# Guoxs/DODT

Measured on AMD Instinct MI355X. Metric: frame-pairs/sec (whole node) KITTI-shape tau=2, higher is better.
Workload: dtype f32

## Files before the change

dodt_amd/_lib.py:

```python
import ctypes as C
import os

_HERE = os.path.dirname(os.path.abspath(__file__))
LIB_PATH = os.environ.get('DODT_HIP_LIB') or os.path.join(_HERE, 'lib', 'libdodt_hip.so')

OK, ERR_INVALID, ERR_HIP, ERR_UNSUPPORTED = 0, 1, 2, 3
PTS_VELO_XYZI, PTS_CAM_3XN = 0, 1
EXTRACTOR_VGG_PYR = 0
EXTRACTOR_VGG = 1
EXTRACTOR_SHARED_GPU = 0x100
EXTRACTOR_BF16 = 0x200
EXTRACTOR_SPLIT = 0x400
FC_RELU = 1
FC_BF16 = 2
CONFLICT_RAISE, CONFLICT_NEXT_BEST = 0, 1


class DodtError(RuntimeError):
    pass


class BevParams(C.Structure):
    _fields_ = [
        ('point_format', C.c_int32),
# ... 82 lines not shown
                                      _pf, _pf, _pf]),
    'dodt_project_anchors_f32': (_i, [_vp, _pf, _i, _pi32, C.POINTER(_f),
                                      C.POINTER(_f), _f, _f, _pf, _pf, _pf]),
    'dodt_img_preprocess': (_i, [_vp, _vp, _i, _i, _i, _i, _i,
                                 C.POINTER(_f), _pf]),
    'dodt_conv_mode': (_i, []),
    'dodt_extractor_create': (_i, [_vp, _i, _i, _i, _i, _i, _i,
                                   C.POINTER(_vp)]),
    'dodt_extractor_destroy': (_i, [_vp]),
    'dodt_extractor_set_layer': (_i, [_vp, C.c_char_p, _vp, _i, _i, _i, _i,
                                      _vp, _vp, _vp]),
    'dodt_extractor_input': (_i, [_vp, C.POINTER(_vp), C.POINTER(C.c_longlong)]),
    'dodt_extractor_forward': (_i, [_vp, _pf, _pf, _pf]),
    'dodt_extractor_forward_padded': (_i, [_vp, _pf, _pf, _pf]),
    'dodt_extractor_set_input': (_i, [_vp, _pf]),
    'dodt_extractor_set_input_support': (_i, [_vp, _vp, _i, _i, C.POINTER(C.c_longlong)]),
    'dodt_extractor_set_frame_tables': (_i, [_vp, _i, C.POINTER(_i)]),
    'dodt_extractor_frame_items': (_i, [_vp, C.POINTER(_i), _i]),
    'dodt_extractor_frame_split': (_i, [_vp, C.POINTER(_i), C.POINTER(_i), _i]),
    'dodt_extractor_store_bytes': (C.c_longlong, [_vp]),
    'dodt_frame_tables_host': (_i, [_vp, _i, _i, _i, _i, _i, _i, _vp, _i, _vp, _vp, C.POINTER(_i)]),
    'dodt_frame_restore_host': (_i, [_vp, _i, _i, _i, _i, _i, _i, _i, _i, _i, _vp, _vp, _vp, _vp]),
    'dodt_frame_lists_host': (_i, [_vp, _i, _i, _i, _i, _i, _i, _vp, _i, _vp, _vp, C.POINTER(_i), _vp, C.POINTER(_i)]),
    'dodt_extractor_read_activation': (_i, [_vp, C.c_char_p, _vp,
                                            C.POINTER(_i), C.POINTER(_i),
                                            C.POINTER(_i)]),
    'dodt_extractor_output_shape': (_i, [_vp, C.POINTER(_i), C.POINTER(_i), C.POINTER(_i)]),
    'dodt_extractor_first_layers_folded': (_i, [_vp]),
    'dodt_extractor_flops': (_d, [_vp]),
    'dodt_extractor_mfma_flops': (_d, [_vp]),
    'dodt_extractor_bytes': (_d, [_vp]),
    'dodt_extractor_layer_count': (_i, [_vp]),
    'dodt_conv_variant_count': (_i, []),
    'dodt_conv_variant_info': (_i, [_i, C.POINTER(ConvVariant)]),
    'dodt_conv_plan_host': (_i, [_i, _i, _i, _i, _i, _i, _i, C.POINTER(ConvLayerPlan), _i, C.POINTER(_i)]),
    'dodt_extractor_layer_plan': (_i, [_vp, C.POINTER(ConvLayerPlan), _i, C.POINTER(_i)]),
    'dodt_extractor_forward_timed': (_i, [_vp, _pf, _pf, _pf, C.POINTER(LayerInfo), _i]),
    'dodt_crop_and_resize': (_i, [_vp, _pf, _i, _i, _i, _pf, _i, _pi32, _i, _i,
                                  _pf]),
    'dodt_crop_and_resize_strided': (_i, [_vp, _pf, _i, _i, _i, _pf, _i, _pi32, _i, _i, _pf,
                                          C.c_longlong]),
    'dodt_correlation': (_i, [_vp, _pf, _pf, _i, _i, _i, _i, _i, _i, _pf]),
    'dodt_crop_and_resize_indexed': (_i, [_vp, _pf, _i, _i, _i, _pf, _i, _pi32, _i, _pi32, _i, _i, _pf,
                                          C.c_longlong]),
    'dodt_correlation_tile_list': (_i, [_vp, _i, _i, _pf, _i, _pi32, _i, _pi32, _i, _i, _pi32, _i, _pi32]),
    'dodt_correlation_tiles': (_i, [_vp, _pf, _pf, _i, _i, _i, _i, _i, _i, _pi32, _i, _pi32, _pf]),
    'dodt_mean_fusion': (_i, [_vp, _pf, _pf, _i, _pi32, _i, _pf]),
    'dodt_fc_create': (_i, [_vp, _i, _i, _hf, _hf, _i, C.POINTER(_vp)]),
    'dodt_fc_create_ex': (_i, [_vp, _i, _i, _hf, _hf, _i, C.POINTER(_vp)]),
    'dodt_fc_destroy': (_i, [_vp]),
    'dodt_fc_forward': (_i, [_vp, _vp, _pf, _pf, _i, _i, _pi32, _pf, _i]),
    'dodt_fc_forward_split': (_i, [_vp, _vp, _pf, _i, _i, _pi32, _i, C.POINTER(_i), C.POINTER(_vp)]),
    'dodt_fc_flops': (_d, [_vp, _i]),
    'dodt_fc_bf16_row_elems': (_i, [_vp]),
    'dodt_fc_forward_bf16': (_i, [_vp, _vp, _vp, _i, _i, _pi32, _vp, _i, _i]),
    'dodt_fc_forward_split_bf16': (_i, [_vp, _vp, _vp, _i, _i, _pi32, _i, C.POINTER(_i), C.POINTER(_vp)]),
    'dodt_rows_to_bf16': (_i, [_vp, _pf, _pf, _i, _pi32, _i, _i, _vp, _i]),
    'dodt_nms': (_i, [_vp, _pf, _pf, _i, _pi32, _i, _f, _pi32, _pi32]),
    'dodt_offset_to_anchor': (_i, [_vp, _pf, _pf, _i, _pi32, _pf]),
    'dodt_softmax_fg': (_i, [_vp, _pf, _i, _pi32, _pf]),
    'dodt_rpn_decode': (_i, [_vp, _pf, _pf, _pf, _i, _pi32, C.POINTER(_f), _pf, _pf, _pf]),
    'dodt_gather_project': (_i, [_vp, _pf, _pi32, _i, _pi32, C.POINTER(_f), C.POINTER(_f), _f, _f, _pf, _pf, _pf]),
    'dodt_final_decode': (_i, [_vp, _pf, _pf, _pf, _pf, _i, _pi32, C.POINTER(_f), C.POINTER(_f),
                               _pf, _pf, _pf, _pf, _pf, _pf]),
    'dodt_gather_rows': (_i, [_vp, _pf, _i, _pi32, _i, _pi32, _pf]),
    'dodt_max_fg_logit': (_i, [_vp, _pf, _i, _i, _pi32, _pf]),
    'dodt_pack_detections': (_i, [_vp, _pf, _pf, _pf, _pf, _pi32, _pi32, _i, _f, _pf, _pi32]),
    'dodt_pack_detections_compact': (_i, [_vp, _pf, _pf, _pf, _pf, _pi32, _pi32, _i, _f, _pf, _pi32]),
    'dodt_angle_vector_to_orientation': (_i, [_vp, _pf, _i, _pi32, _pf]),
    'dodt_class_scores': (_i, [_vp, _pf, _i, _i, _pi32, _pf, _pi32]),
    'dodt_final_decode_classes': (_i, [_vp, _pf, _pf, _pf, _i, _pf, _i, _pi32, C.POINTER(_f), C.POINTER(_f),
                                       _pf, _pf, _pf, _pf, _pf, _pi32, _pf]),
    'dodt_pack_detections_classes': (_i, [_vp, _pf, _pf, _pi32, _pf, _pf, _pi32, _pi32, _i, _f, _pf, _pi32]),
    'dodt_pack_detections_compact_classes': (_i, [_vp, _pf, _pf, _pi32, _pf, _pf, _pi32, _pi32, _i, _f, _pf, _pi32]),
    'dodt_box_4c_decode': (_i, [_vp, _pf, _pf, _i, _pi32, C.POINTER(_f),
                                C.POINTER(_f), _pf, _pf, _pf]),
    'dodt_comm_unique_id': (_i, [_vp]),
    'dodt_comm_create': (_i, [_vp, _i, _i, _vp, C.POINTER(_vp)]),
    'dodt_comm_destroy': (_i, [_vp]),
    'dodt_comm_attach': (_i, [_vp, _vp]),
    'dodt_comm_rank': (_i, [_vp, C.POINTER(_i), C.POINTER(_i)]),
    'dodt_comm_set_late_peer': (_i, [_vp, _d]),
    'dodt_all_gather_records': (_i, [_vp, _vp, _i, _pf, _pi32, _i, _i, _i, _i, _pf, _pi32]),
    'dodt_comm_join': (_i, [_vp, _i, _vp]),
    'dodt_comm_sync': (_i, [_vp]),
    'dodt_comm_barrier': (_i, [_vp]),
    'dodt_comm_max_f64': (_i, [_vp, C.POINTER(_d)]),
    'dodt_three_d_iou_matrix': (_i, [_vp, _vp, _i, _vp, _i, _vp]),
    'dodt_interpolate_pairs': (_i, [_vp, _vp, _i, _pi32, _i, _i, _i, _d, _i, _vp, C.POINTER(_d), _i, _vp,
                                    _pi32, _pi32]),
    'dodt_track_state_bytes': (_i, [_i, C.POINTER(C.c_size_t)]),
    'dodt_track_reset': (_i, [_vp, _vp, _i]),
    'dodt_track_flush': (_i, [_vp, _vp, _d, _i]),
    'dodt_track_encode': (_i, [_vp, _vp, _i, _pi32, _i, _i, C.POINTER(_d), _d, _d, _d, _pf, _pf, _pi32]),
    'dodt_track_pairs': (_i, [_vp, _vp, _vp, _i, _pi32, _i, _i, C.POINTER(_d), _d, _d, _d, _d, _d, _i]),
    'dodt_track_encoded': (_i, [_vp, _vp, _pf, _pf, _pi32, _i, _i, _d, _d, _i]),
}
COMM_ID_BYTES = 128

_lib = None


def load():
    global _lib
    if _lib is not None:
        return _lib
# ... 21 lines not shown
```

dodt_amd/csrc/gemm.hip:

```cpp
#include <cmath>
#include <cstdlib>
#include <mutex>
#include <set>
#include <type_traits>
#include <vector>

#include <algorithm>

#include "common.h"
#include "lds_dma.h"

namespace {

typedef float f32x16 __attribute__((ext_vector_type(16)));
typedef float f32x4 __attribute__((ext_vector_type(4)));

constexpr int kKAlign = 64;
constexpr int kSmallK = 16;

struct GemmArgs {
    const float* x;
    const float* x2;
    const float* w;
    const float* bias;
// ... 347 lines not shown
                wf[q][nt] = *reinterpret_cast<const f32x4*>(sS + w_base + q * (2 * kDmaBN * 4) + nt * 128);
            if (FUSE) x2[q] = *reinterpret_cast<const f32x4*>(sS + kDmaXFloats + xo[q]);
        };
        read_q(0);
        read_q(1);
        __builtin_amdgcn_sched_barrier(0);
        constexpr int kPerQ = (kPerStage + 3) / 4;
#pragma unroll
        for (int q = 0; q < 4; ++q) {
            if (q + 2 < 4) read_q(q + 2);
            if (FUSE) {
#pragma unroll
                for (int e = 0; e < 4; ++e) xf[q][e] = (xf[q][e] + x2[q][e]) / 2.0f;
            }
#pragma unroll
            for (int s2 = 0; s2 < 4; ++s2)
#pragma unroll
                for (int nt = 0; nt < NT; ++nt)
                    acc[nt] = __builtin_amdgcn_mfma_f32_32x32x2f32(xf[q][s2], wf[q][nt][s2], acc[nt], 0, 0, 0);
            if (more) {
#pragma unroll
                for (int n = q * kPerQ; n < (q + 1) * kPerQ && n < kPerStage; ++n) issue_one(st + 2, (BUF + 2) % kDmaStages, n);
            }
            __builtin_amdgcn_sched_barrier(0);
        }
    };
    auto issue = [&](int st, int buf) {
#pragma unroll
        for (int n = 0; n < kPerStage; ++n) issue_one(st, buf, n);
    };
    issue(0, 0);
    if (nstages > 1) issue(1, 1);
    for (int st = 0; st < nstages; st += 3) {
        stage(std::integral_constant<int, 0>{}, st);
        if (st + 1 < nstages) stage(std::integral_constant<int, 1>{}, st + 1);
        if (st + 2 < nstages) stage(std::integral_constant<int, 2>{}, st + 2);
    }
#pragma unroll
    for (int nt = 0; nt < NT; ++nt) {
        const int n = n0 + wn * 32 * NT + nt * 32 + li;
        store_tile32<false>(a, acc[nt], a.bias[n], m0 + wm * 32 + 4 * lh, n, M);
    }
}

int launch_fc_dma(hipStream_t s, const GemmArgs& a, int Npad, int nt) {
    const int tiles_m = dodt::ceil_div(a.M, kDmaBM), tiles_n = Npad / (64 * nt);
    const dim3 grid(tiles_m * tiles_n);
    const size_t x_floats = (size_t)kDmaXFloats * (a.x2 ? 2 : 1);
    const size_t lds = kDmaStages * (x_floats + (size_t)kDmaBK * 64 * nt) * sizeof(float);
    hipError_t e;
    if (a.x2) e = launch_with_lds(&fc_dma_kernel<true, 1>, grid, lds, s, a, tiles_m, tiles_n);
    else if (nt == 2) e = launch_with_lds(&fc_dma_kernel<false, 2>, grid, lds, s, a, tiles_m, tiles_n);
    else e = launch_with_lds(&fc_dma_kernel<false, 1>, grid, lds, s, a, tiles_m, tiles_n);
    DODT_HIP_CHECK(e);
    DODT_LAUNCH_CHECK();
    return DODT_OK;
}

constexpr int kBfBM = 64, kBfBN = 128, kBfStages = 3;
__host__ __device__ constexpr int bf_swz(int r, int S) { return (r / (16 / S)) & (S - 1); }

template <bool YBF16, int BK>
__global__ void __launch_bounds__(256, 2)
fc_bf16_dma_kernel(const GemmArgs a, int tiles_m, int tiles_n) {
    static_assert(kBfStages == 3, "the stage loop is unrolled for a ring of three");
    using dodt::i32x4_t;
    using dodt::kOob;
    using dodt::make_rsrc;
    constexpr int S = BK / 8;
    constexpr int kXBytes = kBfBM * BK * 2, kWBytes = kBfBN * BK * 2, kStage = kXBytes + kWBytes;
    constexpr int kXPieces = kXBytes / 1024 / 4, kWPieces = kWBytes / 1024 / 4;
    constexpr int kPerStage = kXPieces + kWPieces;
    static_assert(kPerStage <= 63, "vmcnt is six bits");
    constexpr int kRowsPerPiece = 1024 / (BK * 2);
    constexpr int NQ = BK / 16;
    extern __shared__ __attribute__((aligned(16))) float smem[];
    const int tid = threadIdx.x, lane = tid & 63;
    const int wave = __builtin_amdgcn_readfirstlane(tid >> 6);
    const int wm = wave >> 1, wn = wave & 1;
    const int li = lane & 31, lh = lane >> 5;
    const int tile = xcd_tile(tiles_m * tiles_n);
    const int mt = tile / tiles_n, nt0 = tile % tiles_n;
    const int m0 = mt * kBfBM;
    const int M = resolved_rows(a.d_m, a.M);
    if (m0 >= M) return;
    const int nstages = a.Kp / BK;
    const int rows = min(M - m0, kBfBM);
    const unsigned short* x16 = reinterpret_cast<const unsigned short*>(a.x);
    const i32x4_t x_rsrc = make_rsrc(x16 + (size_t)m0 * a.ldx, (unsigned)(((size_t)(rows - 1) * a.ldx + a.Kp) * 2));
    const char* wblk = reinterpret_cast<const char*>(a.w) + (size_t)nt0 * nstages * kWBytes;
    const i32x4_t w_rsrc = make_rsrc(wblk, (unsigned)((size_t)nstages * kWBytes));
    int x_off[kXPieces];
#pragma unroll
    for (int k = 0; k < kXPieces; ++k) {
        const int row = (wave + 4 * k) * kRowsPerPiece + lane / S, slot = (lane % S) ^ bf_swz(row, S);
        x_off[k] = row < rows ? (row * a.ldx + slot * 8) * 2 : kOob;
    }
    const int w_off = lane * 16;
    const unsigned lds0 = (unsigned)(size_t)(__attribute__((address_space(3))) void*)smem;
    auto issue_one = [&](int st, int buf, int n) {
        const unsigned sX = lds0 + (unsigned)(buf * kStage);
        if (n < kXPieces) dodt::blds16s(x_rsrc, x_off[n < kXPieces ? n : 0], st * (BK * 2), sX + (unsigned)(wave + 4 * n) * 1024);
        else dodt::blds16s(w_rsrc, w_off, st * kWBytes + (wave + 4 * (n - kXPieces)) * 1024,
                           sX + kXBytes + (unsigned)(wave + 4 * (n - kXPieces)) * 1024);
    };
    f32x16 acc[2];
// ... 284 lines not shown
                t = a[(size_t)r * in_ld + c + e];
                if (b) t = (t + b[(size_t)r * in_ld + c + e]) / 2.0f;
            }
            v[e] = t;
        }
        f32x2 o = {pack_bf16(v[0], v[1]), pack_bf16(v[2], v[3])};
        *reinterpret_cast<f32x2*>(out + (size_t)r * out_ld + c) = o;
    }
}
}

extern "C" int dodt_rows_to_bf16(dodt_ctx* ctx, const float* d_a, const float* d_b, int rows, const int32_t* d_n,
                                 int row_floats, int in_ld, void* d_out_bf16, int out_ld) {
    DODT_REQUIRE(ctx && d_a && d_out_bf16, "dodt_rows_to_bf16: NULL argument");
    DODT_REQUIRE(rows >= 0 && row_floats >= 1 && in_ld >= row_floats && out_ld >= row_floats && out_ld % 4 == 0,
                 "dodt_rows_to_bf16: rows of %d floats, %d apart, into rows of %d bf16 (a multiple of 4)", row_floats,
                 in_ld, out_ld);
    DODT_REQUIRE((size_t)d_out_bf16 % 8 == 0, "dodt_rows_to_bf16: 8-byte aligned output");
    if (rows == 0) return DODT_OK;
    const long long total = (long long)rows * (out_ld / 4);
    const int blocks = (int)std::min<long long>((total + 255) / 256, 4096);
    hipLaunchKernelGGL(rows_to_bf16_kernel, dim3(blocks), dim3(256), 0, ctx->stream, d_a, d_b, rows, d_n, row_floats,
                       in_ld, reinterpret_cast<unsigned short*>(d_out_bf16), out_ld);
    DODT_LAUNCH_CHECK();
    return DODT_OK;
}

struct dodt_fc {
    dodt_ctx* ctx = nullptr;
    int K = 0, Kp = 0, N = 0, Npad = 0, BN = 0, relu = 0;
    bool bf16 = false;
    float* d_w = nullptr;
    float* d_b = nullptr;
    float* d_w_plain = nullptr;
    void* d_w_dma = nullptr;
    int Kd = 0;
    int dma_bk = 0;
    bool smallk = false;
    bool skinny = false;
    bool dma = false;
};

namespace {

enum class FcForm {
    kNone,
    kSmallK,
    kSkinny,
    kSkinnyBf16,
    kSkinnyBf16Rows,
    kDmaNt1,
    kDmaNt2,
    kDmaFused,
    kBf16RowsDma32,
    kBf16RowsDma64,
    kTiled64x128,
    kTiled128x32,
    kTiled64x128Bf16,
    kTiled128x32Bf16,
};

FcForm select_fc_form(const dodt_fc& f, const GemmArgs& a, bool x_bf16, bool y_bf16) {
    if (x_bf16) {
        if (f.d_w_dma) return f.dma_bk == 64 ? FcForm::kBf16RowsDma64 : FcForm::kBf16RowsDma32;
        if (f.skinny && a.ldx % 4 == 0 && (size_t)a.x % 8 == 0 && !y_bf16) return FcForm::kSkinnyBf16Rows;
        return FcForm::kNone;
    }
    if (f.smallk && (size_t)a.y % 16 == 0) return FcForm::kSmallK;
    if (f.skinny && a.ldx % 4 == 0 && (size_t)a.x % 16 == 0 && !a.x2) return f.bf16 ? FcForm::kSkinnyBf16 : FcForm::kSkinny;
    if (f.bf16) {
        return f.BN == 128 ? FcForm::kTiled64x128Bf16 : FcForm::kTiled128x32Bf16;
    }
    if (f.BN != 128) return FcForm::kTiled128x32;
    if (f.dma && a.ldx % 4 == 0 && (size_t)a.x % 16 == 0 && (!a.x2 || (size_t)a.x2 % 16 == 0)) {
        if (a.x2) return FcForm::kDmaFused;
        const long tiles128 = (long)dodt::ceil_div(a.M, kDmaBM) * (f.Npad / 128);
        return tiles128 >= 2 * 256 ? FcForm::kDmaNt2 : FcForm::kDmaNt1;
    }
    return FcForm::kTiled64x128;
}

int launch_fc_form(FcForm form, const dodt_fc& f, hipStream_t s, GemmArgs a, const SplitOut& so, bool y_bf16) {
    switch (form) {
    case FcForm::kSmallK: return launch_fc_smallk(s, a, f.d_w_plain, f.bf16);
    case FcForm::kSkinny: return launch_fc_skinny(s, a, so, false, false);
    case FcForm::kSkinnyBf16: return launch_fc_skinny(s, a, so, true, false);
    case FcForm::kSkinnyBf16Rows: return launch_fc_skinny(s, a, so, true, true);
    case FcForm::kDmaNt1:
    case FcForm::kDmaFused: return launch_fc_dma(s, a, f.Npad, 1);
    case FcForm::kDmaNt2: return launch_fc_dma(s, a, f.Npad, 2);
    case FcForm::kBf16RowsDma32:
    case FcForm::kBf16RowsDma64:
        a.w = reinterpret_cast<const float*>(f.d_w_dma);
        a.Kp = f.Kd;
        return launch_fc_bf16_dma(s, a, f.Npad, y_bf16, f.dma_bk);
    case FcForm::kTiled64x128: return launch_fc<64, 128, 2, 2, 64, false>(s, a, f.Npad);
    case FcForm::kTiled128x32: return launch_fc<128, 32, 4, 1, 32, false>(s, a, f.Npad);
    case FcForm::kTiled64x128Bf16: return launch_fc<64, 128, 2, 2, 32, true>(s, a, f.Npad);
    case FcForm::kTiled128x32Bf16: return launch_fc<128, 32, 4, 1, 64, true>(s, a, f.Npad);
    case FcForm::kNone: break;
    }
    dodt::set_error("dodt_fc: no kernel form selected");
    return DODT_ERR_UNSUPPORTED;
}

GemmArgs fc_args(const dodt_fc& f, const void* d_x, const float* d_x2, int ldx, int M, const int32_t* d_m, void* d_y,
                 int ldy) {
    GemmArgs a;
    a.x = reinterpret_cast<const float*>(d_x); a.x2 = d_x2; a.w = f.d_w; a.bias = f.d_b; a.y = reinterpret_cast<float*>(d_y);
    a.M = M; a.K = f.K; a.Kp = f.Kp; a.N = f.N; a.ldx = ldx; a.ldy = ldy; a.relu = f.relu;
    a.d_m = d_m;
    return a;
}

SplitOut whole_out(const dodt_fc& f, void* d_y, int ldy) {
    float* y = reinterpret_cast<float*>(d_y);
    return SplitOut{{y, y, y}, {f.N, f.N, f.N}, {ldy, ldy, ldy}};
}

int split_out(const char* who, const dodt_fc& f, int parts, const int* widths, float* const* d_ys, SplitOut* so) {
    int end = 0;
    for (int p = 0; p < 3; ++p) {
        const int q = p < parts ? p : parts - 1;
        DODT_REQUIRE(widths[q] >= 1 && d_ys[q], "%s: part %d is empty", who, q);
        if (p < parts) end += widths[p];
        so->y[p] = d_ys[q];
        so->n_end[p] = p < parts ? end : f.N + 1;
        so->ld[p] = widths[q];
    }
    DODT_REQUIRE(end == f.N, "%s: the parts have %d columns, the layer %d", who, end, f.N);
    return DODT_OK;
}

}

extern "C" {

int dodt_fc_create(dodt_ctx* ctx, int K, int N, const float* w, const float* bias, int relu,
                   dodt_fc** out) {
    return dodt_fc_create_ex(ctx, K, N, w, bias, relu ? DODT_FC_RELU : 0, out);
}

int dodt_fc_create_ex(dodt_ctx* ctx, int K, int N, const float* w, const float* bias, int flags,
// ... 107 lines not shown
        dodt::set_error("dodt_fc_forward_split: layers with N <= 32, K %% 16 == 0 and 16-byte aligned rows only");
        return DODT_ERR_UNSUPPORTED;
    }
    if (M == 0) return DODT_OK;
    return launch_fc_form(form, *f, (ctx ? ctx : f->ctx)->stream, a, so, false);
}

int dodt_fc_bf16_row_elems(const dodt_fc* f) {
    if (!f || !f->bf16) return 0;
    if (f->d_w_dma) return f->Kd;
    return f->skinny ? f->K : 0;
}

int dodt_fc_forward_bf16(dodt_fc* f, dodt_ctx* ctx, const void* d_x_bf16, int ldx, int M, const int32_t* d_m,
                         void* d_y, int ldy, int y_bf16) {
    DODT_REQUIRE(f && d_x_bf16 && d_y, "dodt_fc_forward_bf16: NULL argument");
    DODT_REQUIRE(f->bf16, "dodt_fc_forward_bf16: the layer was not created with DODT_FC_BF16");
    DODT_REQUIRE(M >= 0 && ldy >= f->N, "dodt_fc_forward_bf16: bad strides");
    if (M == 0) return DODT_OK;
    const GemmArgs a = fc_args(*f, d_x_bf16, nullptr, ldx, M, d_m, d_y, ldy);
    const FcForm form = select_fc_form(*f, a, true, y_bf16 != 0);
    if (form == FcForm::kBf16RowsDma32 || form == FcForm::kBf16RowsDma64) {
        DODT_REQUIRE(ldx >= f->Kd && ldx % 8 == 0 && (size_t)d_x_bf16 % 16 == 0,
                     "dodt_fc_forward_bf16: rows of >= %d bf16 (zeros beyond K = %d), 16-byte aligned", f->Kd, f->K);
        DODT_REQUIRE((size_t)M * ldx * 2 < (1ull << 31), "dodt_fc_forward_bf16: x block beyond 2 GB");
    } else if (form == FcForm::kSkinnyBf16Rows) {
        DODT_REQUIRE(ldx >= f->K, "dodt_fc_forward_bf16: bad strides");
    } else {
        dodt::set_error("dodt_fc_forward_bf16: layers with N %% 128 == 0 and K >= 128, or N <= 32 and K %% 16 == 0 with "
                        "float32 output, only (K = %d, N = %d)", f->K, f->N);
        return DODT_ERR_UNSUPPORTED;
    }
    return launch_fc_form(form, *f, (ctx ? ctx : f->ctx)->stream, a, whole_out(*f, d_y, ldy), y_bf16 != 0);
}

int dodt_fc_forward_split_bf16(dodt_fc* f, dodt_ctx* ctx, const void* d_x_bf16, int ldx, int M, const int32_t* d_m,
                               int parts, const int* widths, float* const* d_ys) {
    DODT_REQUIRE(f && d_x_bf16 && widths && d_ys, "dodt_fc_forward_split_bf16: NULL argument");
    DODT_REQUIRE(f->bf16, "dodt_fc_forward_split_bf16: the layer was not created with DODT_FC_BF16");
    DODT_REQUIRE(parts >= 1 && parts <= 3, "dodt_fc_forward_split_bf16: %d parts (1..3)", parts);
    DODT_REQUIRE(M >= 0 && ldx >= f->K, "dodt_fc_forward_split_bf16: bad strides");
    const GemmArgs a = fc_args(*f, d_x_bf16, nullptr, ldx, M, d_m, nullptr, 0);
    SplitOut so;
    if (int rc = split_out("dodt_fc_forward_split_bf16", *f, parts, widths, d_ys, &so)) return rc;
    const FcForm form = select_fc_form(*f, a, true, false);
    if (form != FcForm::kSkinnyBf16Rows) {
        dodt::set_error("dodt_fc_forward_split_bf16: layers with N <= 32, K %% 16 == 0 and 8-byte aligned rows only");
        return DODT_ERR_UNSUPPORTED;
    }
    if (M == 0) return DODT_OK;
    return launch_fc_form(form, *f, (ctx ? ctx : f->ctx)->stream, a, so, false);
}

double dodt_fc_flops(const dodt_fc* f, int M) {
    return f ? 2.0 * M * (double)f->K * f->N : 0.0;
}

}
```

dodt_amd/ops.py:

```python
import ctypes as C

import numpy as np

from dodt_amd import _lib


def _arr(ctype, values):
    values = [float(v) for v in np.asarray(values, dtype=np.float64).reshape(-1)]
    return (ctype * len(values))(*values)


def _p(a):
    return None if a is None else C.c_void_p(a.ptr)


def make_bev_params(cfg, velo_to_cam=None, p2=None, im_wh=None,
                    point_format=_lib.PTS_VELO_XYZI, ground_plane=None,
                    area_extents=None, voxel_size=None):
    bp = _lib.BevParams()
    bp.point_format = point_format
    bp.num_slices = int(cfg['num_slices'])
    m = np.zeros(12) if velo_to_cam is None else \
        np.asarray(velo_to_cam, dtype=np.float64).reshape(-1)[:12]
    p = np.zeros(12) if p2 is None else np.asarray(p2, dtype=np.float64).reshape(-1)
# ... 307 lines not shown

    def __init__(self, ctx, w, b, relu, dtype='f32'):
        if dtype not in ('f32', 'bf16'):
            raise ValueError("dtype must be 'f32' or 'bf16'")
        w = np.ascontiguousarray(w, dtype=np.float32)
        b = np.ascontiguousarray(b, dtype=np.float32)
        if w.ndim != 2 or b.shape != (w.shape[1],):
            raise ValueError('weights must be (K,N) and bias (N,)')
        self.ctx, self.K, self.N, self.dtype = ctx, int(w.shape[0]), int(w.shape[1]), dtype
        h = C.c_void_p()
        flags = (_lib.FC_RELU if relu else 0) | (_lib.FC_BF16 if dtype == 'bf16' else 0)
        _lib.check(ctx.lib.dodt_fc_create_ex(ctx.handle, self.K, self.N,
                                             w.ctypes.data_as(C.c_void_p),
                                             b.ctypes.data_as(C.c_void_p), flags, C.byref(h)),
                   'dodt_fc_create_ex')
        self.handle = h

    def forward(self, d_x, M, d_y, ldx=None, ldy=None, d_x2=None, d_m=None, ctx=None):
        c = ctx or self.ctx
        _lib.check(c.lib.dodt_fc_forward(
            self.handle, c.handle, _p(d_x), _p(d_x2), int(self.K if ldx is None else ldx),
            int(M), _p(d_m), _p(d_y), int(self.N if ldy is None else ldy)), 'dodt_fc_forward')

    def can_split(self, ldx=None):
        return self.N <= 32 and self.K % 16 == 0 and (self.K if ldx is None else ldx) % 4 == 0

    def forward_split(self, d_x, M, d_ys, widths, ldx=None, d_m=None, ctx=None):
        c = ctx or self.ctx
        w = (C.c_int * len(widths))(*[int(v) for v in widths])
        ys = (C.c_void_p * len(d_ys))(*[_p(y) for y in d_ys])
        _lib.check(c.lib.dodt_fc_forward_split(
            self.handle, c.handle, _p(d_x), int(self.K if ldx is None else ldx), int(M), _p(d_m),
            len(widths), w, ys), 'dodt_fc_forward_split')

    def bf16_row_elems(self):
        return int(self.ctx.lib.dodt_fc_bf16_row_elems(self.handle)) if self.dtype == 'bf16' else 0

    def forward_bf16(self, d_x, M, d_y, ldx, ldy=None, d_m=None, y_bf16=True, ctx=None):
        c = ctx or self.ctx
        _lib.check(c.lib.dodt_fc_forward_bf16(self.handle, c.handle, _p(d_x), int(ldx), int(M), _p(d_m), _p(d_y),
                                              int(self.N if ldy is None else ldy), 1 if y_bf16 else 0),
                   'dodt_fc_forward_bf16')

    def forward_split_bf16(self, d_x, M, d_ys, widths, ldx, d_m=None, ctx=None):
        c = ctx or self.ctx
        w = (C.c_int * len(widths))(*[int(v) for v in widths])
        ys = (C.c_void_p * len(d_ys))(*[_p(y) for y in d_ys])
        _lib.check(c.lib.dodt_fc_forward_split_bf16(
            self.handle, c.handle, _p(d_x), int(ldx), int(M), _p(d_m), len(widths), w, ys), 'dodt_fc_forward_split_bf16')

    def flops(self, M):
        return 2.0 * M * self.K * self.N

    def close(self):
        if self.handle is not None:
            self.ctx.lib.dodt_fc_destroy(self.handle)
            self.handle = None


def three_d_iou_matrix(ctx, d_a, na, d_b, nb, d_iou_out):
    _lib.check(ctx.lib.dodt_three_d_iou_matrix(ctx.handle, _p(d_a), int(na), _p(d_b), int(nb), _p(d_iou_out)),
               'dodt_three_d_iou_matrix')


def temporal_calib(r0_rect, tr_velo_to_cam):
    r0 = np.asarray(r0_rect, np.float64).reshape(3, 3)
    tr = np.asarray(tr_velo_to_cam, np.float64).reshape(3, 4)
    inv = np.zeros_like(tr)
    inv[0:3, 0:3] = np.transpose(tr[0:3, 0:3])
    inv[0:3, 3] = np.dot(-np.transpose(tr[0:3, 0:3]), tr[0:3, 3])
    return np.concatenate([np.linalg.inv(r0).reshape(-1), inv.reshape(-1), tr.reshape(-1), r0.reshape(-1)])


def temporal_ego(ego, n_frames):
    if len(ego) != n_frames - 1:
        raise ValueError('recovery needs one (trans, matrix, delta) per frame 1..n_frames-1')
    out = np.zeros((n_frames, 13))
    for i, (trans, matrix, delta) in enumerate(ego):
        out[i + 1, 0:3] = np.asarray(trans, np.float64).reshape(3)
        out[i + 1, 3:12] = np.linalg.inv(np.asarray(matrix, np.float64).reshape(3, 3)).reshape(-1)
        out[i + 1, 12] = float(delta)
    return out


def interpolate_pairs(ctx, d_records, d_counts, n_pairs, max_det, n_frames, threshold, on_conflict, d_out,
                      d_out_counts, d_status, d_recover=None, calib=None, max_out=None):
    if on_conflict not in ('raise', 'next_best'):
        raise ValueError("on_conflict must be 'raise' or 'next_best'")
    if d_records.dtype not in (np.float32, np.float64):
        raise ValueError('records must be float32 or float64')
    cal = None if calib is None else _arr(C.c_double, calib)
    _lib.check(ctx.lib.dodt_interpolate_pairs(
        ctx.handle, _p(d_records), int(d_records.dtype == np.float64), _p(d_counts), int(n_pairs), int(max_det),
        int(n_frames), float(threshold), _lib.CONFLICT_NEXT_BEST if on_conflict == 'next_best' else _lib.CONFLICT_RAISE,
        _p(d_recover), cal, int(2 * max_det if max_out is None else max_out), _p(d_out), _p(d_out_counts),
        _p(d_status)), 'dodt_interpolate_pairs')


def track_state_bytes(log_capacity):
    n = C.c_size_t()
    _lib.check(_lib.load().dodt_track_state_bytes(int(log_capacity), C.byref(n)), 'dodt_track_state_bytes')
    return int(n.value)


def track_reset(ctx, d_state, log_capacity):
    _lib.check(ctx.lib.dodt_track_reset(ctx.handle, _p(d_state), int(log_capacity)), 'dodt_track_reset')
# ... 31 lines not shown
```

include/dodt_hip.h:

```cpp
#ifndef DODT_HIP_H
#define DODT_HIP_H

#include <stddef.h>
#include <stdint.h>

#ifdef __cplusplus
extern "C" {
#endif

#define DODT_OK 0
#define DODT_ERR_INVALID 1
#define DODT_ERR_HIP 2
#define DODT_ERR_UNSUPPORTED 3

typedef struct dodt_ctx dodt_ctx;

int dodt_version(void);
const char* dodt_last_error(void);
int dodt_ctx_create(int device_id, dodt_ctx** out);
int dodt_ctx_create_high_priority(int device_id, dodt_ctx** out);
int dodt_ctx_create_on_stream(int device_id, void* hip_stream, dodt_ctx** out);
int dodt_ctx_destroy(dodt_ctx* ctx);
int dodt_ctx_set_plan_cus(dodt_ctx* ctx, int n);
int dodt_ctx_sync(dodt_ctx* ctx);
// ... 147 lines not shown
    int32_t pool_fused;
    int32_t bneck_fused;
    int32_t folded;
    int32_t reserved_;
} dodt_conv_layer_plan;
int dodt_conv_plan_host(int kind, int in_h, int in_w, int in_c, int pad_top, int batch, int num_cus,
                        dodt_conv_layer_plan* out, int n_out, int* n_layers);
int dodt_extractor_layer_plan(const dodt_extractor* ex, dodt_conv_layer_plan* out, int n_out, int* n_layers);
int dodt_extractor_forward_timed(dodt_extractor* ex, const float* d_in, float* d_feat_out,
                                 float* d_bottleneck_out, dodt_layer_info* info, int n_info);

int dodt_crop_and_resize(dodt_ctx* ctx, const float* d_image, int H, int W, int C,
                         const float* d_boxes, int n, const int32_t* d_n, int crop_h,
                         int crop_w, float* d_out);
int dodt_crop_and_resize_strided(dodt_ctx* ctx, const float* d_image, int H, int W, int C,
                                 const float* d_boxes, int n, const int32_t* d_n, int crop_h,
                                 int crop_w, float* d_out, long long out_box_stride);
int dodt_crop_and_resize_indexed(dodt_ctx* ctx, const float* d_image, int H, int W, int C,
                                 const float* d_boxes, int n_boxes, const int32_t* d_box_idx, int n,
                                 const int32_t* d_n, int crop_h, int crop_w, float* d_out,
                                 long long out_box_stride);

int dodt_correlation(dodt_ctx* ctx, const float* d_a, const float* d_b, int H, int W, int C,
                     int max_displacement, int stride_2, int pad, float* d_out);
int dodt_correlation_tile_list(dodt_ctx* ctx, int OH, int OW, const float* d_boxes, int n_boxes,
                               const int32_t* d_box_idx, int n, const int32_t* d_n, int crop_h, int crop_w,
                               int32_t* d_tiles, int capacity, int32_t* d_n_tiles);
int dodt_correlation_tiles(dodt_ctx* ctx, const float* d_a, const float* d_b, int H, int W, int C,
                           int max_displacement, int stride_2, int pad, const int32_t* d_tiles, int capacity,
                           const int32_t* d_n_tiles, float* d_out);

int dodt_mean_fusion(dodt_ctx* ctx, const float* d_a, const float* d_b, int rows, const int32_t* d_n,
                     int row_floats, float* d_out);
typedef struct dodt_fc dodt_fc;
int dodt_fc_create(dodt_ctx* ctx, int K, int N, const float* w, const float* bias, int relu,
                   dodt_fc** out);
#define DODT_FC_RELU 1
#define DODT_FC_BF16 2
int dodt_fc_create_ex(dodt_ctx* ctx, int K, int N, const float* w, const float* bias, int flags,
                      dodt_fc** out);
int dodt_fc_destroy(dodt_fc* fc);
int dodt_fc_forward(dodt_fc* fc, dodt_ctx* ctx, const float* d_x, const float* d_x2, int ldx,
                    int M, const int32_t* d_m, float* d_y, int ldy);
int dodt_fc_forward_split(dodt_fc* fc, dodt_ctx* ctx, const float* d_x, int ldx, int M, const int32_t* d_m,
                          int parts, const int* widths, float* const* d_ys);
int dodt_fc_bf16_row_elems(const dodt_fc* fc);
int dodt_fc_forward_bf16(dodt_fc* fc, dodt_ctx* ctx, const void* d_x_bf16, int ldx, int M, const int32_t* d_m,
                         void* d_y, int ldy, int y_bf16);
int dodt_fc_forward_split_bf16(dodt_fc* fc, dodt_ctx* ctx, const void* d_x_bf16, int ldx, int M, const int32_t* d_m,
                               int parts, const int* widths, float* const* d_ys);
int dodt_rows_to_bf16(dodt_ctx* ctx, const float* d_a, const float* d_b, int rows, const int32_t* d_n,
                      int row_floats, int in_ld, void* d_out_bf16, int out_ld);
double dodt_fc_flops(const dodt_fc* fc, int M);

int dodt_nms(dodt_ctx* ctx, const float* d_boxes, const float* d_scores, int n,
             const int32_t* d_n, int max_out, float iou_threshold, int32_t* d_sel_out,
             int32_t* d_count_out);

int dodt_offset_to_anchor(dodt_ctx* ctx, const float* d_anchors, const float* d_offsets,
                          int n, const int32_t* d_n, float* d_out);
int dodt_softmax_fg(dodt_ctx* ctx, const float* d_logits2, int n, const int32_t* d_n,
                    float* d_scores_out);
int dodt_rpn_decode(dodt_ctx* ctx, const float* d_anchors, const float* d_offsets, const float* d_logits2, int n,
                    const int32_t* d_n, const float bev_extents[4], float* d_regressed_out,
                    float* d_bev_norm_tf_out, float* d_scores_out);
int dodt_gather_project(dodt_ctx* ctx, const float* d_src, const int32_t* d_idx, int n, const int32_t* d_n,
                        const float bev_extents[4], const float p2[12], float im_w, float im_h,
                        float* d_rows_out, float* d_bev_norm_tf_out, float* d_img_norm_tf_out);
int dodt_final_decode(dodt_ctx* ctx, const float* d_top_anchors, const float* d_offsets, const float* d_cls_logits2,
                      const float* d_angle_vectors, int n, const int32_t* d_n, const float plane[4],
                      const float bev_extents[4], float* d_boxes_3d_out, float* d_pred_anchors_out,
                      float* d_bev_tf_out, float* d_nms_scores_out, float* d_det_scores_out,
                      float* d_orientations_out);
int dodt_gather_rows(dodt_ctx* ctx, const float* d_src, int width, const int32_t* d_idx,
                     int n, const int32_t* d_n, float* d_out);
int dodt_max_fg_logit(dodt_ctx* ctx, const float* d_logits, int n_cls, int n,
                      const int32_t* d_n, float* d_scores_out);
int dodt_angle_vector_to_orientation(dodt_ctx* ctx, const float* d_angle_vectors, int n,
                                     const int32_t* d_n, float* d_orientations_out);
int dodt_pack_detections(dodt_ctx* ctx, const float* d_boxes_3d, const float* d_scores,
                         const float* d_orientations, const float* d_corr_offsets,
                         const int32_t* d_sel, const int32_t* d_count, int max_det,
                         float frame_mark, float* d_rec_out, int32_t* d_count_out);
int dodt_pack_detections_compact(dodt_ctx* ctx, const float* d_boxes_3d, const float* d_scores,
                                 const float* d_orientations, const float* d_det_offsets,
                                 const int32_t* d_sel, const int32_t* d_count, int max_det,
                                 float frame_mark, float* d_rec_out, int32_t* d_count_out);
int dodt_class_scores(dodt_ctx* ctx, const float* d_logits, int n_cls, int n, const int32_t* d_n,
                      float* d_scores_out, int32_t* d_types_out);
int dodt_final_decode_classes(dodt_ctx* ctx, const float* d_top_anchors, const float* d_offsets,
                              const float* d_cls_logits, int n_cls, const float* d_angle_vectors, int n,
                              const int32_t* d_n, const float plane[4], const float bev_extents[4],
                              float* d_boxes_3d_out, float* d_pred_anchors_out, float* d_bev_tf_out,
                              float* d_nms_scores_out, float* d_det_scores_out, int32_t* d_det_types_out,
                              float* d_orientations_out);
int dodt_pack_detections_classes(dodt_ctx* ctx, const float* d_boxes_3d, const float* d_scores, const int32_t* d_types,
                                 const float* d_orientations, const float* d_corr_offsets, const int32_t* d_sel,
                                 const int32_t* d_count, int max_det, float frame_mark, float* d_rec_out,
                                 int32_t* d_count_out);
int dodt_pack_detections_compact_classes(dodt_ctx* ctx, const float* d_boxes_3d, const float* d_scores,
                                         const int32_t* d_types, const float* d_orientations,
                                         const float* d_det_offsets, const int32_t* d_sel, const int32_t* d_count,
                                         int max_det, float frame_mark, float* d_rec_out, int32_t* d_count_out);
int dodt_box_4c_decode(dodt_ctx* ctx, const float* d_top_anchors, const float* d_offsets,
                       int n, const int32_t* d_n, const float plane[4],
                       const float bev_extents[4], float* d_boxes_3d_out,
// ... 46 lines not shown
```

Measured before the change: 420.8.

## Add small-M DMA FC kernel tiling N into 16-wide blocks

Adds an f32 FC kernel for M up to 128 rows. It launches one workgroup per 16 output columns, streams X and W through a four-stage LDS ring using buffer-to-LDS DMA, and runs 16x16x4 f32 MFMAs. Form selection now routes unfused DMA-eligible calls with small M to this kernel. The goal is to fill the GPU with many more workgroups than the 64-row tiled DMA path gives for small batches. In exchange, each block re-reads the whole X slab and the waitcnt bookkeeping is hand-tuned. A form-name query is also exposed for diagnostics.

```diff
diff --git a/dodt_amd/_lib.py b/dodt_amd/_lib.py
--- a/dodt_amd/_lib.py
+++ b/dodt_amd/_lib.py
@@ -158,6 +158,7 @@
     'dodt_fc_forward': (_i, [_vp, _vp, _pf, _pf, _i, _i, _pi32, _pf, _i]),
     'dodt_fc_forward_split': (_i, [_vp, _vp, _pf, _i, _i, _pi32, _i, C.POINTER(_i), C.POINTER(_vp)]),
     'dodt_fc_flops': (_d, [_vp, _i]),
+    'dodt_fc_form_name': (C.c_char_p, [_vp, _i, _i, _i, _i]),
     'dodt_fc_bf16_row_elems': (_i, [_vp]),
     'dodt_fc_forward_bf16': (_i, [_vp, _vp, _vp, _i, _i, _pi32, _vp, _i, _i]),
     'dodt_fc_forward_split_bf16': (_i, [_vp, _vp, _vp, _i, _i, _pi32, _i, C.POINTER(_i), C.POINTER(_vp)]),
diff --git a/dodt_amd/csrc/gemm.hip b/dodt_amd/csrc/gemm.hip
--- a/dodt_amd/csrc/gemm.hip
+++ b/dodt_amd/csrc/gemm.hip
@@ -423,6 +423,155 @@
     if (a.x2) e = launch_with_lds(&fc_dma_kernel<true, 1>, grid, lds, s, a, tiles_m, tiles_n);
     else if (nt == 2) e = launch_with_lds(&fc_dma_kernel<false, 2>, grid, lds, s, a, tiles_m, tiles_n);
     else e = launch_with_lds(&fc_dma_kernel<false, 1>, grid, lds, s, a, tiles_m, tiles_n);
+    DODT_HIP_CHECK(e);
+    DODT_LAUNCH_CHECK();
+    return DODT_OK;
+}
+
+constexpr int kSmBM = 128, kSmBN = 16, kSmBK = 16, kSmStages = 4;
+constexpr int kSmXFloats = kSmBM * kSmBK, kSmWFloats = kSmBK * kSmBN;
+constexpr int kSmStage = kSmXFloats + kSmWFloats;
+__host__ __device__ constexpr int sm_swz(int row) { return (-(row >> 2)) & 3; }
+
+__global__ void __launch_bounds__(256) __attribute__((amdgpu_waves_per_eu(8)))
+fc_dma_small_m_kernel(const GemmArgs a) {
+    static_assert(kSmStages == 4, "the stage loop is unrolled for a ring of four");
+    using dodt::i32x4_t;
+    using dodt::kOob;
+    using dodt::make_rsrc;
+    extern __shared__ __attribute__((aligned(16))) float smem[];
+    const int tid = threadIdx.x, lane = tid & 63;
+    const int wave = __builtin_amdgcn_readfirstlane(tid >> 6);
+    const int li = lane & 15, lg = lane >> 4;
+    const int rows = min(resolved_rows(a.d_m, a.M), kSmBM);
+    if (rows <= 0) return;
+    const int nstages = a.K / kSmBK, last = nstages - 1;
+    const int n0 = blockIdx.x * kSmBN;
+
+    const i32x4_t x_rsrc = make_rsrc(a.x, (unsigned)(((size_t)(rows - 1) * a.ldx + a.K) * 4));
+    const float* wblk = a.w + ((size_t)(n0 / 128) * (a.Kp / 8) * 2 * 128 + (n0 % 128)) * 4;
+    const i32x4_t w_rsrc = make_rsrc(wblk, (unsigned)(((size_t)(a.Kp / 8) * 2 * 128 - (n0 % 128)) * 16));
+    int x_off[2];
+#pragma unroll
+    for (int k = 0; k < 2; ++k) {
+        const int row = (wave + 4 * k) * 16 + (lane >> 2), cq = (lane & 3) ^ sm_swz(row);
+        x_off[k] = row < rows ? (row * a.ldx + cq * 4) * 4 : kOob;
+    }
+    const int w_off = (lg * 128 + li) * 16;
+    const unsigned lds0 = (unsigned)(size_t)(__attribute__((address_space(3))) void*)smem;
+    auto issue_one = [&](int st, int buf, int n) {
+        const unsigned sX = lds0 + (unsigned)(buf * kSmStage) * 4;
+        if (n < 2) dodt::blds16s(x_rsrc, x_off[n], st * (kSmBK * 4), sX + (unsigned)(wave + 4 * n) * 1024);
+        else if (wave == 0) dodt::blds16s(w_rsrc, w_off, st * (4 * 128 * 16), sX + kSmXFloats * 4);
+    };
+    auto issue = [&](int st, int buf) {
+#pragma unroll
+        for (int n = 0; n < 3; ++n) issue_one(st, buf, n);
+    };
+    auto wait_ahead = [&](int ahead) {
+        if (ahead >= 3) {
+            if (wave == 0) __builtin_amdgcn_s_waitcnt(0x0f70 | 9);
+            else __builtin_amdgcn_s_waitcnt(0x0f70 | 6);
+        } else if (ahead == 2) {
+            if (wave == 0) __builtin_amdgcn_s_waitcnt(0x0f70 | 6);
+            else __builtin_amdgcn_s_waitcnt(0x0f70 | 4);
+        } else if (ahead == 1) {
+            if (wave == 0) __builtin_amdgcn_s_waitcnt(0x0f70 | 3);
+            else __builtin_amdgcn_s_waitcnt(0x0f70 | 2);
+        } else {
+            __builtin_amdgcn_s_waitcnt(0x0f70);
+        }
+    };
+
+    int xo[2];
+#pragma unroll
+    for (int qb = 0; qb < 2; ++qb)
+        xo[qb] = (wave * 32 + li) * kSmBK + (((2 * qb + (lg & 1)) ^ sm_swz(li)) * 4);
+    const int wo = kSmXFloats + ((lg & 1) * kSmBN + li) * 4;
+    const unsigned pick_sel = lane >= 32 ? 0x07060504u : 0x03020100u;
+    auto pick = [&](float even, float odd) {
+        return __builtin_bit_cast(float, __builtin_amdgcn_perm(__builtin_bit_cast(unsigned, odd),
+                                                               __builtin_bit_cast(unsigned, even), pick_sel));
+    };
+
+    f32x4 acc[2] = {{0.f, 0.f, 0.f, 0.f}, {0.f, 0.f, 0.f, 0.f}};
+    f32x4 xr[2], wr;
+    float xa[2][2][2], wb[2][2];
+    auto read_block = [&](int buf, int qb) {
+        const float* sS = smem + buf * kSmStage;
+#pragma unroll
+        for (int t = 0; t < 2; ++t) xr[t] = *reinterpret_cast<const f32x4*>(sS + xo[qb] + t * (16 * kSmBK));
+        wr = *reinterpret_cast<const f32x4*>(sS + wo + qb * (2 * kSmBN * 4));
+    };
+    auto select_block = [&](int qb) {
+#pragma unroll
+        for (int j = 0; j < 2; ++j) {
+#pragma unroll
+            for (int t = 0; t < 2; ++t) xa[t][qb][j] = pick(xr[t][2 * j], xr[t][2 * j + 1]);
+            wb[qb][j] = pick(wr[2 * j], wr[2 * j + 1]);
+        }
+    };
+    auto stage = [&](auto bufc, auto morec, auto nextc, int st) {
+        const int buf = bufc;
+        const bool more = morec, next = nextc;
+        const int nbuf = buf + 1 < kSmStages ? buf + 1 : buf + 1 - kSmStages;
+        if (next) {
+            wait_ahead(more ? kSmStages - 2 : min(kSmStages - 2, last - st - 1));
+            __builtin_amdgcn_s_barrier();
+        }
+#pragma unroll
+        for (int qb = 0; qb < 2; ++qb) {
+            if (next) read_block(nbuf, qb);
+            __builtin_amdgcn_sched_barrier(0);
+#pragma unroll
+            for (int j = 0; j < 2; ++j) {
+#pragma unroll
+                for (int t = 0; t < 2; ++t)
+                    acc[t] = __builtin_amdgcn_mfma_f32_16x16x4f32(xa[t][qb][j], wb[qb][j], acc[t], 0, 0, 0);
+                if (more && 2 * qb + j < 3) issue_one(st + kSmStages, buf, 2 * qb + j);
+                __builtin_amdgcn_sched_barrier(0);
+            }
+            if (next) select_block(qb);
+            __builtin_amdgcn_sched_barrier(0);
+        }
+    };
+#pragma unroll
+    for (int b = 0; b < kSmStages; ++b)
+        if (b < nstages) issue(b, b);
+    wait_ahead(min(kSmStages - 1, last));
+    __builtin_amdgcn_s_barrier();
+#pragma unroll
+    for (int qb = 0; qb < 2; ++qb) {
+        read_block(0, qb);
+        select_block(qb);
+    }
+    const int nmore = nstages - kSmStages;
+    int st = 0;
+    for (; st + kSmStages <= nmore; st += kSmStages) {
+        stage(std::integral_constant<int, 0>{}, std::true_type{}, std::true_type{}, st);
+        stage(std::integral_constant<int, 1>{}, std::true_type{}, std::true_type{}, st + 1);
+        stage(std::integral_constant<int, 2>{}, std::true_type{}, std::true_type{}, st + 2);
+        stage(std::integral_constant<int, 3>{}, std::true_type{}, std::true_type{}, st + 3);
+    }
+    for (int buf = 0; st < nstages; ++st, buf = buf + 1 < kSmStages ? buf + 1 : 0) stage(buf, st < nmore, st < last, st);
+    const int n = n0 + li;
+    const float b = a.bias[n];
+#pragma unroll
+    for (int t = 0; t < 2; ++t)
+#pragma unroll
+        for (int r = 0; r < 4; ++r) {
+            const int m = wave * 32 + t * 16 + 4 * lg + r;
+            if (m < rows && n < a.N) {
+                float v = acc[t][r] + b;
+                if (a.relu) v = fmaxf(v, 0.0f);
+                a.y[(size_t)m * a.ldy + n] = v;
+            }
+        }
+}
+
+int launch_fc_dma_small_m(hipStream_t s, const GemmArgs& a, int Npad) {
+    const size_t lds = (size_t)kSmStages * kSmStage * sizeof(float);
+    hipError_t e = launch_with_lds(&fc_dma_small_m_kernel, dim3(Npad / kSmBN), lds, s, a);
     DODT_HIP_CHECK(e);
     DODT_LAUNCH_CHECK();
     return DODT_OK;
@@ -813,6 +962,7 @@
     kDmaNt1,
     kDmaNt2,
     kDmaFused,
+    kDmaSmallM,
     kBf16RowsDma32,
     kBf16RowsDma64,
     kTiled64x128,
@@ -835,6 +985,7 @@
     if (f.BN != 128) return FcForm::kTiled128x32;
     if (f.dma && a.ldx % 4 == 0 && (size_t)a.x % 16 == 0 && (!a.x2 || (size_t)a.x2 % 16 == 0)) {
         if (a.x2) return FcForm::kDmaFused;
+        if (a.M <= kSmBM) return FcForm::kDmaSmallM;
         const long tiles128 = (long)dodt::ceil_div(a.M, kDmaBM) * (f.Npad / 128);
         return tiles128 >= 2 * 256 ? FcForm::kDmaNt2 : FcForm::kDmaNt1;
     }
@@ -850,6 +1001,7 @@
     case FcForm::kDmaNt1:
     case FcForm::kDmaFused: return launch_fc_dma(s, a, f.Npad, 1);
     case FcForm::kDmaNt2: return launch_fc_dma(s, a, f.Npad, 2);
+    case FcForm::kDmaSmallM: return launch_fc_dma_small_m(s, a, f.Npad);
     case FcForm::kBf16RowsDma32:
     case FcForm::kBf16RowsDma64:
         a.w = reinterpret_cast<const float*>(f.d_w_dma);
@@ -1063,6 +1215,31 @@
     return launch_fc_form(form, *f, (ctx ? ctx : f->ctx)->stream, a, so, false);
 }
 
+const char* dodt_fc_form_name(const dodt_fc* f, int M, int ldx, int two_inputs, int x_bf16) {
+    if (!f) return "none";
+    const float* aligned = reinterpret_cast<const float*>((size_t)256);
+    const GemmArgs a = fc_args(*f, aligned, two_inputs ? aligned : nullptr, ldx, M, nullptr,
+                               const_cast<float*>(aligned), f->N);
+    switch (select_fc_form(*f, a, x_bf16 != 0, false)) {
+    case FcForm::kNone: return "none";
+    case FcForm::kSmallK: return "smallk";
+    case FcForm::kSkinny: return "skinny";
+    case FcForm::kSkinnyBf16: return "skinny_bf16";
+    case FcForm::kSkinnyBf16Rows: return "skinny_bf16_rows";
+    case FcForm::kDmaNt1: return "dma_64x64";
+    case FcForm::kDmaNt2: return "dma_64x128";
+    case FcForm::kDmaFused: return "dma_fused";
+    case FcForm::kDmaSmallM: return "dma_small_m";
+    case FcForm::kBf16RowsDma32: return "bf16_rows_dma32";
+    case FcForm::kBf16RowsDma64: return "bf16_rows_dma64";
+    case FcForm::kTiled64x128: return "tiled_64x128";
+    case FcForm::kTiled128x32: return "tiled_128x32";
+    case FcForm::kTiled64x128Bf16: return "tiled_64x128_bf16";
+    case FcForm::kTiled128x32Bf16: return "tiled_128x32_bf16";
+    }
+    return "none";
+}
+
 double dodt_fc_flops(const dodt_fc* f, int M) {
     return f ? 2.0 * M * (double)f->K * f->N : 0.0;
 }
diff --git a/dodt_amd/ops.py b/dodt_amd/ops.py
--- a/dodt_amd/ops.py
+++ b/dodt_amd/ops.py
@@ -383,6 +383,10 @@
     def flops(self, M):
         return 2.0 * M * self.K * self.N
 
+    def form_name(self, M, ldx=None, two_inputs=False, x_bf16=False):
+        return self.ctx.lib.dodt_fc_form_name(self.handle, int(M), int(self.K if ldx is None else ldx),
+                                              1 if two_inputs else 0, 1 if x_bf16 else 0).decode()
+
     def close(self):
         if self.handle is not None:
             self.ctx.lib.dodt_fc_destroy(self.handle)
diff --git a/include/dodt_hip.h b/include/dodt_hip.h
--- a/include/dodt_hip.h
+++ b/include/dodt_hip.h
@@ -223,6 +223,7 @@
 int dodt_rows_to_bf16(dodt_ctx* ctx, const float* d_a, const float* d_b, int rows, const int32_t* d_n,
                       int row_floats, int in_ld, void* d_out_bf16, int out_ld);
 double dodt_fc_flops(const dodt_fc* fc, int M);
+const char* dodt_fc_form_name(const dodt_fc* fc, int M, int ldx, int two_inputs, int x_bf16);
 
 int dodt_nms(dodt_ctx* ctx, const float* d_boxes, const float* d_scores, int n,
              const int32_t* d_n, int max_out, float iou_threshold, int32_t* d_sel_out,
```

Result: no change. 424.0 (median of 6 runs) (+0.8%).
